# oxli-bio/oxli

Hardware: NVIDIA B200
Metric: canonical k-mers counted/sec (higher is better)
Workload: dtype u64

## Files before the change

oxli_b200/csrc/capi.cu:

```cuda
#include <algorithm>
#include <atomic>
#include <cerrno>
#include <chrono>
#include <cmath>
#include <cstdarg>
#include <cstddef>
#include <condition_variable>
#include <cstdio>
#include <cstdlib>
#include <cstring>
#include <functional>
#include <memory>
#include <mutex>
#include <string>
#include <system_error>
#include <thread>
#include <vector>

#include <fcntl.h>
#include <unistd.h>

#include <cuda_runtime.h>
#include <nvtx3/nvToolsExt.h>

// ... 262 lines not shown
}

int grid_for(const DeviceCtx *c, uint64_t items, int threads, int per_sm) {
    uint64_t want = (items + threads - 1) / threads;
    return (int)std::max<uint64_t>(1, std::min<uint64_t>(want, (uint64_t)c->sms * per_sm));
}

constexpr uint64_t kSparseBytes = 128ull << 20;
uint64_t capacity_for_keys(uint64_t keys);
bool over_loaded(uint64_t size, uint64_t cap) {
    if (cap * 16 < kSparseBytes) return size * 10 > cap * 3;
    return size * 10 > cap * 7;
}

uint64_t pow2_at_least(uint64_t x) {
    uint64_t c = kMinCap;
    while (c < x) c <<= 1;
    return c;
}

uint64_t capacity_for_keys(uint64_t keys) {
    uint64_t cap = pow2_at_least(keys + keys / 2 + 1);
    while (cap * 16 < kSparseBytes && keys * 10 > cap * 3) cap <<= 1;
    return cap;
}

uint64_t slots_for(uint64_t keys) { return std::max(capacity_for_keys(keys), pow2_at_least(keys * 2)); }

oxg_status free_device_bytes(size_t *free_b) {
    size_t total = 0;
    CU(cudaMemGetInfo(free_b, &total));
    return OXG_OK;
}

oxg_status larger_and_fits(uint64_t keys, uint64_t cap, bool *yes) {
    *yes = false;
    const uint64_t want = slots_for(keys);
    if (want <= cap) return OXG_OK;
    size_t free_b = 0;
    TRY(free_device_bytes(&free_b));
    *yes = want * 16 < free_b / 2;
    return OXG_OK;
}


}

namespace {
struct PartPlan {
    uint32_t n_parts = 0, part_bits = 0;
    int n_ranks = 1, self_rank = 0, owner_shift = 64;
    uint32_t grid_a = 0;
    uint32_t frag_cap = 0;
    uint32_t line_shift = 4;
    uint64_t spill_cap = 0;
    uint32_t groups = 1;
    uint32_t n_dest() const { return n_parts * (uint32_t)n_ranks; }
    uint64_t frag_entries() const { return (uint64_t)n_dest() * grid_a * frag_cap; }
};

}

struct oxg_table {
    DeviceCtx *ctx = nullptr;
    uint32_t k = 0;
    ulonglong2 *slots = nullptr;
    uint64_t cap = 0;
    Ctrl *d_ctrl = nullptr;
    Ctrl *h_ctrl = nullptr;
    uint64_t size = 0;
    bool hinted = false;
    uint64_t hint_keys = 0;
    bool pooled = false;
    float last_ms_a = 0.f, last_ms_b = 0.f;
    struct {
        bool active = false;
        PartPlan pl;
        uint32_t launches = 0;
        uint64_t windows = 0, planned = 0;
    } pend;
    uint64_t part_budget = 0;
    uint32_t group_cap = 0;
    uint32_t *d_sketch = nullptr;
    uint32_t *h_sketch = nullptr;
    uint64_t sketch_covers = 0;
    uint64_t est_keys = 0;
    uint64_t last_made = 0;
    uint64_t last_new = 0;
    float last_ms = 0.f;
    uint64_t last_launches = 0;
};

namespace {

TableView view_of(const oxg_table *t, const DeferLists *defer = nullptr) {
    TableView v;
    v.slots = t->slots;
    v.cap = t->cap;
    uint32_t lg = 0;
    while ((1ull << lg) < t->cap) ++lg;
    v.shift = 64 - lg;
    v.limit = t->cap - t->cap / 5;
    v.ctrl = t->d_ctrl;
    v.overflow = defer ? defer->d_pairs : nullptr;
    v.overflow_cap = defer ? defer->cap : 0;
    return v;
}
// ... 144 lines not shown
}

template <int MODE>
oxg_status launch_consume(oxg_table *t, const ConsumeParams &p) {
    DeviceCtx *c = t->ctx;
    const int k = (int)t->k;
    auto grid_of = [&](const void *fn, size_t smem) {
        int per_sm = 1;
        if (cudaOccupancyMaxActiveBlocksPerMultiprocessor(&per_sm, fn, kThreads, smem) != cudaSuccess || per_sm < 1) per_sm = 1;
        const uint64_t tiles_per_cta = specialised_k(t->k) ? kThreads / 32 : 1;
        const uint64_t work = p.n_tiles;
        return (int)std::max<uint64_t>(1, std::min<uint64_t>((work + tiles_per_cta - 1) / tiles_per_cta, (uint64_t)c->sms * per_sm));
    };
    if (const void *fn = specialised_entry(t->k, MODE)) {
        const size_t dyn = consume_dyn_smem(MODE);
        if (dyn) TRY(max_dyn_smem(fn, c->dev, dyn));
        void *args[] = {const_cast<ConsumeParams *>(&p)};
        CU(cudaLaunchKernel(fn, dim3(grid_of(fn, dyn)), dim3(kThreads), args, dyn, c->stream));
    } else {
        const size_t smem = generic_smem_bytes(k);
        consume_generic_kernel<MODE><<<grid_of((const void *)consume_generic_kernel<MODE>, smem), kThreads, smem, c->stream>>>(p);
    }
    LAUNCHED();
    CU(cudaGetLastError());
    return OXG_OK;
}



uint32_t group_launches(const oxg_table *t) {
    const uint32_t g = g_accumulate.load();
    return t->group_cap ? std::min(g, t->group_cap) : g;
}

bool use_partitioned(const oxg_table *t, uint64_t span) {
    if (!specialised_entry(t->k, kModePart)) return false;
    const int choice = g_pipeline.load();
    if (choice == 1) return false;
    if (choice == 2) return true;
    if (t->pend.active) return true;
    return span >= kPartMinWindows;
}

uint32_t choose_parts(const oxg_table *t, uint32_t max_parts) {
    const uint32_t forced = g_parts_override.load();
    if (forced >= 2 && !(forced & (forced - 1))) return std::min(forced, std::max(max_parts, 2u));
    const uint64_t est = std::max(t->size + t->last_new, t->hint_keys);
    if (est == 0) return std::min<uint32_t>(1024, max_parts);
    uint64_t parts = 64;
    while (parts < max_parts && parts * 6144 < est) parts <<= 1;
    return (uint32_t)std::min<uint64_t>(parts, max_parts);
}

size_t scatter_smem_rt(uint32_t k, uint32_t n_dest, uint32_t line_shift) {
    const uint32_t q = 8 * ((k + 7 + 7) / 8);
    const uint32_t bl = ((kWarpTile - 8 + q) + 15) / 16 * 16;
    return (((size_t)n_dest * ((8u << line_shift) + 12) + 16 + 15) & ~(size_t)15) + (size_t)kScatWarps * (2 * bl + 128);
}

oxg_status plan_partitioned(oxg_table *t, uint64_t span, uint64_t n_tiles, int n_ranks, int self_rank, PartPlan *out) {
    DeviceCtx *c = t->ctx;
    PartPlan pl;
    pl.n_parts = choose_parts(t, std::max(2u, 2048u / (uint32_t)n_ranks));
    while ((1u << pl.part_bits) < pl.n_parts) ++pl.part_bits;
    pl.n_ranks = n_ranks; pl.self_rank = self_rank;
    int lg = 0;
    while ((1 << lg) < n_ranks) ++lg;
    pl.owner_shift = 64 - lg;
    pl.line_shift = 4;
    while (pl.line_shift > 1 && scatter_smem_rt(t->k, pl.n_dest(), pl.line_shift) * kScatCtasPerSm > 220u * 1024) --pl.line_shift;
    if (scatter_smem_rt(t->k, pl.n_dest(), pl.line_shift) * kScatCtasPerSm > 220u * 1024) return fail(OXG_ERR_INVALID, "internal: too many scatter destinations");
    const uint64_t tiles_per_cta = kScatWarps;
    pl.grid_a = (uint32_t)std::max<uint64_t>(1, std::min<uint64_t>((n_tiles + tiles_per_cta - 1) / tiles_per_cta, (uint64_t)c->sms * kScatCtasPerSm));
    const uint64_t line = 1ull << pl.line_shift;
    const uint64_t fair = span / ((uint64_t)pl.n_dest() * pl.grid_a) + 1;
    uint64_t sq = 1;
    while (sq * sq < fair) ++sq;
    pl.frag_cap = (uint32_t)((fair + fair / 2 + 4 * sq + line + line - 1) & ~(line - 1));
    pl.spill_cap = span;
    const uint32_t forced_groups = g_groups_override.load();
    pl.groups = forced_groups ? forced_groups : std::max<uint32_t>(1, std::min<uint32_t>(8, (4u * (uint32_t)c->sms + pl.n_parts - 1) / pl.n_parts));
    if (pl.frag_entries() >> 32) return fail(OXG_ERR_INVALID, "internal: fragment buffer too large for one launch");
    *out = pl;
    return OXG_OK;
}

oxg_status scatter_attr(DeviceCtx *c, uint32_t k) { return max_dyn_smem(specialised_entry(k, kModePart), c->dev, 227 * 1024); }

oxg_status ensure_part_buffers(DeviceCtx *c, const PartPlan &pl) {
    TRY(ensure_dev(&c->d_frag, &c->frag_cap, pl.frag_entries()));
    TRY(ensure_dev(&c->d_frag_cnt, &c->frag_cnt_cap, (uint64_t)pl.n_dest() * pl.grid_a));
    TRY(ensure_dev(&c->d_spill, &c->spill_cap, pl.spill_cap));
    if (!c->d_spill_n) CU(cudaMalloc(&c->d_spill_n, 8));
    return OXG_OK;
}

oxg_status launch_part_a(oxg_table *t, ConsumeParams p, const PartPlan &pl, uint64_t *d_frag, uint32_t *d_frag_cnt,
                         uint64_t *d_spill, unsigned long long *d_spill_n, cudaStream_t stream, bool append = false) {
    DeviceCtx *c = t->ctx;
    const void *fn = specialised_entry(t->k, kModePart);
    TRY(scatter_attr(c, t->k));
    const size_t dyn = scatter_smem_rt(t->k, pl.n_dest(), pl.line_shift);
    p.frag = d_frag; p.frag_cnt = d_frag_cnt; p.frag_cap = pl.frag_cap;
    p.n_parts = pl.n_parts; p.part_shift = 64 - pl.part_bits; p.n_dest = pl.n_dest(); p.line_shift = pl.line_shift;
    p.n_ranks = pl.n_ranks; p.self_rank = pl.self_rank; p.owner_shift = pl.owner_shift;
    p.spill = d_spill; p.spill_cap = pl.spill_cap; p.spill_n = d_spill_n;
    p.frag_append = append ? 1u : 0u;
    if (!append) CU(cudaMemsetAsync(d_spill_n, 0, 8, stream));
    void *args[] = {&p};
    CU(cudaLaunchKernel(fn, dim3(pl.grid_a), dim3(kScatThreads), args, dyn, stream));
    LAUNCHED();
    CU(cudaGetLastError());
    return OXG_OK;
}

constexpr int kAggThreadsDirect = 1024;
const void *const kAggCached = (const void *)aggregate_kernel<kAggThreadsDefault, true>;
const void *const kAggDirect = (const void *)aggregate_kernel<kAggThreadsDirect, false>;

uint32_t use_cache_for(const oxg_table *t, const PartPlan &pl, uint64_t windows) {
    const uint64_t keys = std::max(std::max(t->size, t->hint_keys), t->est_keys);
    return keys == 0 || (windows >= 2 * keys && keys <= 8192ull * pl.n_parts) ? 1u : 0u;
}

uint32_t aggregate_groups(const PartPlan &pl, uint32_t use_cache, uint64_t hashes) {
    if (use_cache || g_groups_override.load()) return pl.groups;
    const uint64_t items = std::max<uint64_t>(1, hashes / 40960);
    return (uint32_t)std::max<uint64_t>(pl.groups, std::min<uint64_t>(64, (items + pl.n_parts - 1) / pl.n_parts));
}

AggParams agg_params(const TableView &v, const PartPlan &pl, const AggSource *src, int n_src) {
    AggParams a{};
    a.table = v;
    for (int s = 0; s < n_src; ++s) a.src[s] = src[s];
    a.n_src = n_src;
    a.n_parts = pl.n_parts; a.dest0 = (uint32_t)pl.self_rank * pl.n_parts; a.n_ctas = pl.grid_a;
    a.frag_cap = pl.frag_cap; a.part_bits = pl.part_bits; a.spill_cap = pl.spill_cap;
    a.owner_shift = pl.owner_shift; a.self_rank = pl.self_rank; a.n_ranks = pl.n_ranks;
    return a;
}

oxg_status launch_part_b(oxg_table *t, const TableView &v, const PartPlan &pl, const AggSource *src, int n_src,
                         uint64_t windows, cudaStream_t stream) {
    DeviceCtx *c = t->ctx;
    AggParams a = agg_params(v, pl, src, n_src);
    a.work_counter = (unsigned long long *)&t->d_ctrl->absorb_counter;
    a.use_cache = use_cache_for(t, pl, windows);
    a.groups = aggregate_groups(pl, a.use_cache, windows);
    const void *fn = a.use_cache ? kAggCached : kAggDirect;
    const int threads = a.use_cache ? kAggThreadsDefault : kAggThreadsDirect;
    const size_t smem = aggregate_smem_bytes(a.use_cache != 0);
    if (a.use_cache) TRY(max_dyn_smem(fn, c->dev, smem));
    int per_sm = 1;
    if (cudaOccupancyMaxActiveBlocksPerMultiprocessor(&per_sm, fn, threads, smem) != cudaSuccess || per_sm < 1) per_sm = 1;
    const uint64_t items = (uint64_t)a.n_parts * a.groups;
    const int grid = (int)std::max<uint64_t>(1, std::min<uint64_t>(items, (uint64_t)c->sms * per_sm));
    void *args[] = {&a};
    CU(cudaLaunchKernel(fn, dim3(grid), dim3(threads), args, smem, stream));
    LAUNCHED();
    CU(cudaGetLastError());
// ... 1097 lines not shown
```

oxli_b200/csrc/capi_shard.inc:

```

constexpr int kSnapRing = 8;

struct oxg_shard {
    oxg_table *table = nullptr;
    DeviceCtx *ctx = nullptr;
    int rank = 0, n_ranks = 1;
    PartPlan plan;
    uint64_t round_windows = 0;
    uint64_t small_round = 0;
    uint64_t batch_windows = 0;
    uint8_t *area = nullptr;
    uint64_t area_bytes = 0;
    uint64_t off_gather = 0, off_cnt[2] = {}, off_spill_n[2] = {}, off_frag[2] = {}, off_spill[2] = {};
    uint8_t *peer[kShardMaxRanks] = {};
    bool peer_ipc[kShardMaxRanks] = {};
    bool connected = false;
    uint64_t rounds_done = 0;
    uint64_t gather_seq = 0;
    uint8_t *d_blob = nullptr;
    uint8_t *h_blob = nullptr;
    Ctrl *h_snap[kSnapRing] = {};
    cudaEvent_t ev_round[kSnapRing] = {};
    uint64_t snaps_seen = 0;
    StageRing ring;
// ... 1000 lines not shown
    return OXG_OK;
}

oxg_status shard_dump(oxg_shard *s, const char *path, int sort_mode) {
    if (!s->connected) return fail(OXG_ERR_INVALID, "shard is not connected to its peers (oxg_shard_connect)");
    if (sort_mode < 0 || sort_mode > 2) return fail(OXG_ERR_INVALID, "sort_mode must be 0, 1 or 2");
    if (!path) return fail(OXG_ERR_INVALID, "null argument");
    CallBufs bufs(s->stream);
    LocalPairs lp;
    LocalText tx;
    std::vector<uint64_t> count, len, bytes, start, at;
    oxg_status st = shard_local_pairs(s, bufs, sort_mode, true, &lp);
    local_runs(lp, sort_mode, &count, &len);
    if (st == OXG_OK) st = shard_text_lengths(s, bufs, lp, len, &tx);
    bytes.assign(len.size(), 0);
    if (st == OXG_OK)
        for (size_t j = 0; j < len.size(); ++j) bytes[j] = tx.bounds[j + 1] - tx.bounds[j];
    uint64_t total_n = 0, total_b = 0;
    TRY(shard_place_runs(s, st, sort_mode, path_hash_of(path), count, len, bytes, &start, &at, &total_n, &total_b));
    TRY(shard_agree(s, s->rank == 0 ? create_sized(path, total_b) : OXG_OK));
    const int fd = open(path, O_WRONLY | O_CLOEXEC);
    if (fd < 0) {
        st = fail(OXG_ERR_IO, "cannot open %s: %s", path, strerror(errno));
    } else {
        st = shard_write_text(s, lp, tx, at, fd, path);
        if (close(fd) != 0 && st == OXG_OK) st = fail(OXG_ERR_IO, "cannot write %s: %s", path, strerror(errno));
    }
    cudaStreamSynchronize(s->ring.copy);
    cudaStreamSynchronize(s->stream);
    return shard_agree(s, st);
}

}

extern "C" {

oxg_status oxg_shard_create(int device, uint32_t ksize, int rank, int n_ranks, uint64_t capacity_hint,
                            uint64_t round_windows, oxg_shard **out) {
    if (!out) return fail(OXG_ERR_INVALID, "out is null");
    *out = nullptr;
    if (n_ranks < 1 || n_ranks > kShardMaxRanks || (n_ranks & (n_ranks - 1)))
        return fail(OXG_ERR_INVALID, "n_ranks must be a power of two in 1..%d", kShardMaxRanks);
    if (rank < 0 || rank >= n_ranks) return fail(OXG_ERR_INVALID, "rank out of range");
    if (!specialised_entry(ksize, kModePart)) return fail(OXG_ERR_INVALID, "a sharded table needs a k with a specialised kernel (csrc/klist.h); got %u", ksize);
    auto s = std::make_unique<oxg_shard>();
    TRY(oxg_table_create(device, ksize, capacity_hint, &s->table));
    oxg_table *t = s->table;
    DeviceCtx *c = t->ctx;
    s->ctx = c; s->rank = rank; s->n_ranks = n_ranks;
    std::lock_guard<std::mutex> lk(c->mu);
    CU(cudaSetDevice(c->dev));
    s->round_windows = round_windows ? round_windows : kLaunchWindows;
    if (s->round_windows < (1u << 16)) s->round_windows = 1u << 16;
    s->round_windows = std::max<uint64_t>(s->round_windows, (uint64_t)c->sms * kScatCtasPerSm * kScatWarps * kWarpTile);
    s->round_windows = align_up(s->round_windows, kWarpTile);
    TRY(plan_partitioned(t, s->round_windows, s->round_windows / kWarpTile + 1, n_ranks, rank, &s->plan));
    if (s->plan.grid_a != (uint32_t)(c->sms * kScatCtasPerSm)) return fail(OXG_ERR_INVALID, "internal: round too small for a full grid");
    if (s->plan.spill_cap < lookup_cap(s.get())) return fail(OXG_ERR_INVALID, "internal: spill region smaller than a merge round");
    shard_layout(s.get());
    CU(cudaMalloc(&s->area, s->area_bytes));
    CU(cudaMemsetAsync(s->area, 0, sizeof(ShardHeader) + (uint64_t)n_ranks * kGatherBytes, c->stream));
    CU(cudaStreamCreateWithFlags(&s->stream, cudaStreamNonBlocking));
    TRY(s->ring.init());
    CU(cudaMalloc(&s->d_blob, kGatherBytes));
    CU(cudaMallocHost(&s->h_blob, (uint64_t)n_ranks * kGatherBytes));
    for (int b = 0; b < kSnapRing; ++b) {
        CU(cudaMallocHost(&s->h_snap[b], sizeof(Ctrl)));
        memset(s->h_snap[b], 0, sizeof(Ctrl));
        CU(cudaEventCreateWithFlags(&s->ev_round[b], cudaEventDisableTiming));
    }
    CU(cudaEventCreate(&s->ev_t0));
    CU(cudaEventCreate(&s->ev_t1));
    s->small_round = align_up(std::max<uint64_t>(std::min<uint64_t>(s->round_windows, kLaunchWindows), (uint64_t)s->plan.grid_a * kScatWarps * kWarpTile), kWarpTile);
    s->small_round = std::min(s->small_round, s->round_windows);
    s->batch_windows = s->round_windows;
    s->defer.cap = s->defer.cap2 = std::max<uint64_t>(kShardDeferCap, 2 * s->small_round);
    s->defer.fixed = true;
    CU(cudaMalloc(&s->defer.d_pairs, s->defer.cap * sizeof(ulonglong2)));
    CU(cudaMalloc(&s->defer.d_pairs2, s->defer.cap2 * sizeof(ulonglong2)));
    t->pooled = true;
    {
        cudaMemPool_t pool;
        CU(cudaDeviceGetDefaultMemPool(&pool, c->dev));
        uint64_t keep = ~0ULL;
        CU(cudaMemPoolSetAttribute(pool, cudaMemPoolAttrReleaseThreshold, &keep));
    }
    TRY(s->ring.reserve(kStageBufs, std::min<uint64_t>(s->round_windows, 4ull << 20) + 256 + 16, false, s->stream));
    for (int b = 0; b < kStageBufs; ++b) TRY(s->ring.reserve_offs(b, 1, s->stream));
    CU(cudaMalloc(&t->d_sketch, kSketchRegs * 4));
    CU(cudaMallocHost(&t->h_sketch, kSketchRegs * 4));
    CU(cudaMemsetAsync(t->d_sketch, 0, kSketchRegs * 4, c->stream));
    s->tile_first_cap = s->round_windows / kWarpTile + 4;
    CU(cudaMalloc(&s->d_tile_first, s->tile_first_cap * 8));
    CU(cudaMalloc(&s->d_bins, (uint64_t)n_ranks * c->sms * kRouteCtasPerSm * 4));
    CU(cudaMallocHost(&s->h_list, kLookupStage * 8));
    TRY(scatter_attr(c, ksize));
    for (const void *fn : {(const void *)route_count_kernel<RouteList>, (const void *)route_count_kernel<RouteSlots>,
                           (const void *)route_scan_kernel, (const void *)route_queries_kernel<RouteList>,
                           (const void *)route_queries_kernel<RouteSlots>, (const void *)answer_queries_kernel,
                           (const void *)gather_answers_kernel, (const void *)apply_pairs_kernel,
                           (const void *)erase_walk_segments_kernel, (const void *)erase_mark_segments_kernel,
                           (const void *)erase_rebuild_kernel, (const void *)cut_kernel, (const void *)init_slots_kernel,
                           (const void *)shard_signal_kernel, (const void *)shard_wait_kernel,
                           (const void *)shard_scatter_blob_kernel, (const void *)stats_kernel,
                           (const void *)export_count_kernel, (const void *)export_scan_kernel,
                           (const void *)export_write_kernel, (const void *)radix_hist_kernel,
                           (const void *)radix_scan_kernel, (const void *)radix_scatter_kernel,
                           (const void *)dump_length_kernel, (const void *)dump_bounds_kernel,
                           (const void *)dump_format_kernel}) {
        cudaFuncAttributes attr;
        CU(cudaFuncGetAttributes(&attr, fn));
    }
    TRY(max_dyn_smem(kAggCached, c->dev, aggregate_smem_bytes(true)));
    CU(cudaStreamSynchronize(c->stream));
    s->peer[rank] = s->area;
    s->connected = n_ranks == 1;
    *out = s.release();
    return OXG_OK;
}

oxg_status oxg_shard_destroy(oxg_shard *s) {
    if (!s) return OXG_OK;
    {
        std::lock_guard<std::mutex> lk(s->ctx->mu);
        cudaSetDevice(s->ctx->dev);
        if (s->d_pos) cudaFreeAsync(s->d_pos, s->stream);
// ... 281 lines not shown
```

oxli_b200/csrc/consume.cuh:

```cuda
#pragma once
#include <utility>

#include "hashing.cuh"
#include "table.cuh"

namespace oxg {

template <class F, int... I>
__device__ __forceinline__ void static_for_impl(F &&f, std::integer_sequence<int, I...>) {
    (f(std::integral_constant<int, I>{}), ...);
}
template <int N, class F>
__device__ __forceinline__ void static_for(F &&f) {
    static_for_impl(f, std::make_integer_sequence<int, N>{});
}

#ifndef OXG_MIN_CTAS
#define OXG_MIN_CTAS 3
#endif

constexpr int kTileW = 2048;
constexpr int kThreads = 256;
constexpr int kWPT = kTileW / kThreads;
static_assert(kWPT == 8, "bit-mask extraction assumes 8 windows per thread");
constexpr int kWarpTile = 32 * kWPT;
constexpr int kMaxRanks = 16;

enum Mode : int {
    kModeCount = 0,
    kModeHash = 1,
    kModeFirstBad = 2,
    kModePart = 3
};

struct ConsumeParams {
    const uint8_t *bases;
    uint64_t g0;
    uint64_t w_lo, w_hi;
    uint64_t data_end;
    uint64_t tile_base;
    uint64_t n_tiles;
    const uint64_t *offsets;
    uint64_t n_off;
    const uint64_t *tile_first;
    TableView table;
    uint64_t *hashes_out;
    uint32_t ksize;
    int owner_shift;
    int self_rank;
    int n_ranks;
    uint64_t *frag;
    uint32_t *frag_cnt;
    uint32_t frag_cap;
    uint32_t n_parts;
    uint32_t part_shift;
    uint32_t n_dest;
    uint32_t line_shift;
    uint32_t frag_append;
    uint64_t *spill;
    uint64_t spill_cap;
    unsigned long long *spill_n;
};

static __global__ void tile_first_kernel(const uint64_t *__restrict__ offsets, uint64_t n_off,
                                  uint64_t tile_base, uint64_t n_tiles, uint32_t tile_w,
                                  uint64_t *__restrict__ tile_first) {
    uint64_t t = blockIdx.x * (uint64_t)blockDim.x + threadIdx.x;
    if (t >= n_tiles) return;
    const uint64_t want = tile_base + t * tile_w + 1;
    uint64_t lo = 0, hi = n_off;
    while (lo < hi) {
        uint64_t mid = (lo + hi) >> 1;
        if (offsets[mid] < want) lo = mid + 1; else hi = mid;
    }
    tile_first[t] = lo;
}

__device__ __forceinline__ uint4 load_bases16(const ConsumeParams &p, uint64_t g) {
    if (g + 16 <= p.data_end) {
        return __ldcs(reinterpret_cast<const uint4 *>(p.bases + (g - p.g0)));
    }
    uint32_t w[4] = {0x4e4e4e4eu, 0x4e4e4e4eu, 0x4e4e4e4eu, 0x4e4e4e4eu};
    for (int b = 0; b < 16; ++b) {
        if (g + b < p.data_end) {
            uint32_t c = p.bases[g + b - p.g0];
            w[b >> 2] = (w[b >> 2] & ~(0xffu << (8 * (b & 3)))) | (c << (8 * (b & 3)));
        }
    }
    return make_uint4(w[0], w[1], w[2], w[3]);
}

template <int BL>
__device__ __forceinline__ void stage16_raw(const ConsumeParams &p, uint64_t w0, int v, uint4 raw, uint8_t *s_fw,
                                            uint8_t *s_rc, uint16_t *s_bad) {
    const uint64_t g = w0 + 16ull * v;
    uint32_t u[4] = {upper4(raw.x), upper4(raw.y), upper4(raw.z), upper4(raw.w)};
    uint32_t ok = acgt_mask4(u[0]) | (acgt_mask4(u[1]) << 4) | (acgt_mask4(u[2]) << 8) |
                  (acgt_mask4(u[3]) << 12);
    if (g + 16 > p.data_end) {
        uint32_t keep = g >= p.data_end ? 0u : (0xffffu >> (16 - (uint32_t)(p.data_end - g)));
        ok &= keep;
    }
    *reinterpret_cast<uint4 *>(s_fw + 16 * v) = make_uint4(u[0], u[1], u[2], u[3]);
    *reinterpret_cast<uint4 *>(s_rc + BL - 16 - 16 * v) =
        make_uint4(bswap32(complement4(u[3])), bswap32(complement4(u[2])),
                   bswap32(complement4(u[1])), bswap32(complement4(u[0])));
    s_bad[v] = (uint16_t)(~ok);
}

template <int BL>
// ... 557 lines not shown
```

oxli_b200/csrc/scatter.cuh:

```cuda
#pragma once
#include "consume.cuh"

namespace oxg {

#ifndef OXG_SCAT_THREADS
#define OXG_SCAT_THREADS 384
#endif
#ifndef OXG_SCAT_CTAS
#define OXG_SCAT_CTAS 2
#endif
constexpr int kScatThreads = OXG_SCAT_THREADS;
constexpr int kScatCtasPerSm = OXG_SCAT_CTAS;
constexpr int kScatWarps = kScatThreads / 32;

template <int K>
struct ScatWarpBuf {
    static constexpr int BL = TileGeom<K>::BL;
    static constexpr int kBytes = 2 * BL + 64 + 64;
};

template <int K>
inline size_t scatter_smem_bytes(uint32_t n_dest, uint32_t line_shift) {
    return (((size_t)n_dest * ((8u << line_shift) + 12) + 16 + 15) & ~(size_t)15) + (size_t)kScatWarps * ScatWarpBuf<K>::kBytes;
}

template <int K>
__global__ void __launch_bounds__(kScatThreads, kScatCtasPerSm) scatter_kernel(const ConsumeParams p) {
    using G = TileGeom<K>;
    constexpr int BL = G::BL, NV = G::NV, NE = G::NE;
    static_assert(NV + 8 <= 32 && NE <= 16, "per-warp mask buffers are 64 bytes each");
    extern __shared__ __align__(128) uint8_t sm[];
    const uint32_t nd = p.n_dest, ls = p.line_shift, line = 1u << ls;
    uint64_t *stage = reinterpret_cast<uint64_t *>(sm);
    uint2 *book = reinterpret_cast<uint2 *>(sm + ((size_t)nd << (ls + 3)));
    uint32_t *flist = reinterpret_cast<uint32_t *>(book + nd);
    uint32_t *s_nflush = flist + nd;
    uint8_t *wbuf = sm + ((((size_t)nd * ((8u << ls) + 12) + 16) + 15) & ~(size_t)15) + (size_t)(threadIdx.x >> 5) * ScatWarpBuf<K>::kBytes;
    uint8_t *s_fw = wbuf, *s_rc = wbuf + BL;
    uint16_t *s_bad = reinterpret_cast<uint16_t *>(wbuf + 2 * BL);
    uint32_t *s_end = reinterpret_cast<uint32_t *>(wbuf + 2 * BL + 64);

    const int lane = threadIdx.x & 31, warp = threadIdx.x >> 5;
    const uint64_t frag_row = (uint64_t)gridDim.x * p.frag_cap;
    uint64_t *const my_frag = p.frag + (uint64_t)blockIdx.x * p.frag_cap;
    for (uint32_t i = threadIdx.x; i < nd; i += kScatThreads) {
        const uint32_t at = p.frag_append ? p.frag_cnt[(uint64_t)i * gridDim.x + blockIdx.x] : 0u;
        book[i] = make_uint2(at, at);
    }
    if (threadIdx.x == 0) *s_nflush = 0;
    __syncthreads();

    auto dest_of = [&](uint64_t h) {
        uint32_t d = (uint32_t)((h * kPhi) >> p.part_shift);
        if (p.n_ranks > 1) d += (uint32_t)(h >> p.owner_shift) * p.n_parts;
        return d;
    };

    uint64_t n_counted = 0, first_bad_unused = ~0ULL;
    const uint64_t tiles_per_round = (uint64_t)gridDim.x * kScatWarps;
    const uint64_t n_rounds = (p.n_tiles + tiles_per_round - 1) / tiles_per_round;
    auto tile_of = [&](uint64_t r) { return (r * gridDim.x + blockIdx.x) * kScatWarps + warp; };

    uint4 raw = make_uint4(0, 0, 0, 0);
    uint64_t tf = 0, off = ~0ULL;
    auto fetch = [&](uint64_t t, uint4 &raw_, uint64_t &tf_) {
        if (t < p.n_tiles) {
            if (lane < NV) raw_ = load_bases16(p, p.tile_base + t * kWarpTile + 16ull * lane);
            tf_ = __ldg(p.tile_first + t);
        }
    };
    auto fetch_off = [&](uint64_t t, uint64_t tf_) {
        const uint64_t rr = tf_ + lane;
        return (t < p.n_tiles && rr < p.n_off) ? __ldg(p.offsets + rr) : ~0ULL;
    };
    fetch(tile_of(0), raw, tf);
    off = fetch_off(tile_of(0), tf);

    const uint32_t lanes_per_line = ls >= 2 ? (line >> 2) : 1u;

    for (uint64_t r = 0; r < n_rounds; ++r) {
        const uint64_t t = tile_of(r);
        uint4 raw_next = make_uint4(0, 0, 0, 0);
        uint64_t tf_next = 0;
        fetch(tile_of(r + 1), raw_next, tf_next);
        uint64_t h[kWPT] = {};
        if (t < p.n_tiles) {
            const uint64_t w0 = p.tile_base + t * kWarpTile;
            if (lane < NE) s_end[lane] = 0;
            __syncwarp();
            if (lane < NV) stage16_raw<BL>(p, w0, lane, raw, s_fw, s_rc, s_bad);
            {
                const uint64_t e = off - 1 - w0;
                if (e < (uint64_t)BL) atomicOr(&s_end[e >> 5], 1u << (e & 31));
                if (__shfl_sync(0xffffffffu, e < (uint64_t)BL, 31)) {
                    for (uint64_t q = tf + 32 + lane; q < p.n_off; q += 32) {
                        const uint64_t e2 = p.offsets[q] - 1 - w0;
                        if (e2 >= (uint64_t)BL) break;
                        atomicOr(&s_end[e2 >> 5], 1u << (e2 & 31));
                    }
                }
            }
            __syncwarp();
            const uint32_t valid = lane_valid_mask<K, kModePart>(p, s_bad, s_end, w0, lane, first_bad_unused);
            if (valid) lane_hashes<K>(s_fw, s_rc, lane * kWPT, valid, h);
        }
        const uint64_t off_next = fetch_off(tile_of(r + 1), tf_next);

        uint32_t dst[kWPT], q[kWPT];
#pragma unroll
        for (int j = 0; j < kWPT; ++j) {
            dst[j] = 0; q[j] = 0;
            if (h[j] != 0) { ++n_counted; dst[j] = dest_of(h[j]); q[j] = atomicAdd(&book[dst[j]].y, 1u); }
        }
        __syncthreads();

        uint32_t later = 0, spilled = 0, last = 0;
        uint2 bk[kWPT];
#pragma unroll
        for (int j = 0; j < kWPT; ++j) bk[j] = book[dst[j]];
#pragma unroll
        for (int j = 0; j < kWPT; ++j) {
            if (h[j] == 0) continue;
            const uint2 b = bk[j];
            const uint32_t total = min(b.y, p.frag_cap), line_end = (b.x & ~(line - 1)) + line;
            if (q[j] >= total) { spilled |= 1u << j; continue; }
            if (q[j] + 1 == total) last |= 1u << j;
            if (q[j] < line_end) {
                stage[((size_t)dst[j] << ls) + (q[j] & (line - 1))] = h[j];
                if (q[j] + 1 == line_end) flist[atomicAdd(s_nflush, 1u)] = dst[j];
            } else if (q[j] < (total & ~(line - 1))) my_frag[dst[j] * frag_row + q[j]] = h[j];
            else later |= 1u << j;
        }
        if (__any_sync(0xffffffffu, spilled != 0)) {
            const uint32_t mine = __popc(spilled);
            uint32_t incl = mine;
            for (int o = 1; o < 32; o <<= 1) {
                const uint32_t v = __shfl_up_sync(0xffffffffu, incl, o);
                if (lane >= o) incl += v;
            }
            const uint32_t tot = __shfl_sync(0xffffffffu, incl, 31);
            unsigned long long base = 0;
            if (lane == 0) base = atomicAdd(p.spill_n, (unsigned long long)tot);
            base = __shfl_sync(0xffffffffu, base, 0) + (incl - mine);
#pragma unroll
            for (int j = 0; j < kWPT; ++j)
                if ((spilled >> j) & 1u) { if (base < p.spill_cap) p.spill[base] = h[j]; ++base; }
        }
        __syncthreads();

        {
            const uint32_t n_flush = *s_nflush;
            if (ls >= 2) {
                const uint32_t per_warp = 32u / lanes_per_line, sub = lane / lanes_per_line, li = (lane % lanes_per_line) * 4;
                for (uint32_t e = warp * per_warp + sub; e < n_flush; e += kScatWarps * per_warp) {
                    const uint32_t d = flist[e];
                    const uint64_t *src = stage + ((size_t)d << ls) + li;
                    const ulonglong2 v0 = *reinterpret_cast<const ulonglong2 *>(src), v1 = *reinterpret_cast<const ulonglong2 *>(src + 2);
                    uint64_t *dstp = my_frag + d * frag_row + (book[d].x & ~(line - 1)) + li;
                    asm volatile("st.global.v4.u64 [%0], {%1,%2,%3,%4};" ::"l"(dstp), "l"(v0.x), "l"(v0.y), "l"(v1.x), "l"(v1.y) : "memory");
                }
            } else {
                const uint32_t per_warp = 32u >> ls, sub = lane >> ls, li = lane & (line - 1);
                for (uint32_t e = warp * per_warp + sub; e < n_flush; e += kScatWarps * per_warp) {
                    const uint32_t d = flist[e];
                    my_frag[d * frag_row + (book[d].x & ~(line - 1)) + li] = stage[((size_t)d << ls) + li];
                }
            }
        }
        __syncthreads();

#pragma unroll
        for (int j = 0; j < kWPT; ++j) {
            if ((later >> j) & 1u) stage[((size_t)dst[j] << ls) + (q[j] & (line - 1))] = h[j];
            if ((last >> j) & 1u) book[dst[j]].x = q[j] + 1;
        }
        if (threadIdx.x == 0) *s_nflush = 0;
        raw = raw_next; tf = tf_next; off = off_next;
    }

    __syncthreads();
    {
        const uint32_t per_warp = 32u >> ls, sub = lane >> ls, li = lane & (line - 1);
        for (uint32_t d = warp * per_warp + sub; d < nd; d += kScatWarps * per_warp) {
            const uint32_t pos = book[d].x, part = pos & (line - 1);
            if (part) my_frag[d * frag_row + (pos - part) + li] = li < part ? stage[((size_t)d << ls) + li] : 0ull;
        }
        for (uint32_t d = threadIdx.x; d < nd; d += kScatThreads)
            p.frag_cnt[(uint64_t)d * gridDim.x + blockIdx.x] = min((book[d].x + line - 1) & ~(line - 1), p.frag_cap);
    }
    for (int o = 16; o; o >>= 1) n_counted += __shfl_xor_sync(0xffffffffu, n_counted, o);
    if (lane == 0 && n_counted) atomicAdd((unsigned long long *)&p.table.ctrl->counted, (unsigned long long)n_counted);
}

}
```

Before: 41.30 billion.

## Replace per-destination line staging with batched counting-sort scatter in pass A

The scatter kernel no longer stages hashes in per-destination shared-memory lines with flush lists. It buffers up to three tiles per warp, counts per destination, prefix-sums the counts across the CTA, and reorders hashes into a shared batch sorted by destination. It then writes them to fragments with contiguous, coalesced stores. This removes the per-round book/line bookkeeping and partial-line padding, at the cost of extra block-wide syncs and a scan per batch, and it caps destinations at 2048 and tiles at 2^31.

```diff
diff --git a/oxli_b200/csrc/capi.cu b/oxli_b200/csrc/capi.cu
--- a/oxli_b200/csrc/capi.cu
+++ b/oxli_b200/csrc/capi.cu
@@ -338,7 +338,7 @@
     int n_ranks = 1, self_rank = 0, owner_shift = 64;
     uint32_t grid_a = 0;
     uint32_t frag_cap = 0;
-    uint32_t line_shift = 4;
+    uint32_t batch_tiles = 1;
     uint64_t spill_cap = 0;
     uint32_t groups = 1;
     uint32_t n_dest() const { return n_parts * (uint32_t)n_ranks; }
@@ -589,10 +589,15 @@
     return (uint32_t)std::min<uint64_t>(parts, max_parts);
 }
 
-size_t scatter_smem_rt(uint32_t k, uint32_t n_dest, uint32_t line_shift) {
+size_t scatter_smem_rt(uint32_t k, uint32_t n_dest, uint32_t batch_tiles) {
     const uint32_t q = 8 * ((k + 7 + 7) / 8);
     const uint32_t bl = ((kWarpTile - 8 + q) + 15) / 16 * 16;
-    return (((size_t)n_dest * ((8u << line_shift) + 12) + 16 + 15) & ~(size_t)15) + (size_t)kScatWarps * (2 * bl + 128);
+    return scatter_smem_bytes(n_dest, batch_tiles, (int)(2 * bl + 128));
+}
+
+uint64_t scatter_full_grid_tiles(const DeviceCtx *c) { return (uint64_t)c->sms * kScatCtasPerSm * kScatWarps; }
+uint32_t scatter_grid(const DeviceCtx *c, uint64_t n_tiles) {
+    return (uint32_t)std::max<uint64_t>(1, std::min<uint64_t>((n_tiles + kScatWarps - 1) / kScatWarps, (uint64_t)c->sms * kScatCtasPerSm));
 }
 
 oxg_status plan_partitioned(oxg_table *t, uint64_t span, uint64_t n_tiles, int n_ranks, int self_rank, PartPlan *out) {
@@ -604,16 +609,15 @@
     int lg = 0;
     while ((1 << lg) < n_ranks) ++lg;
     pl.owner_shift = 64 - lg;
-    pl.line_shift = 4;
-    while (pl.line_shift > 1 && scatter_smem_rt(t->k, pl.n_dest(), pl.line_shift) * kScatCtasPerSm > 220u * 1024) --pl.line_shift;
-    if (scatter_smem_rt(t->k, pl.n_dest(), pl.line_shift) * kScatCtasPerSm > 220u * 1024) return fail(OXG_ERR_INVALID, "internal: too many scatter destinations");
-    const uint64_t tiles_per_cta = kScatWarps;
-    pl.grid_a = (uint32_t)std::max<uint64_t>(1, std::min<uint64_t>((n_tiles + tiles_per_cta - 1) / tiles_per_cta, (uint64_t)c->sms * kScatCtasPerSm));
-    const uint64_t line = 1ull << pl.line_shift;
+    pl.batch_tiles = kScatMaxBatchTiles;
+    while (pl.batch_tiles > 1 && scatter_smem_rt(t->k, pl.n_dest(), pl.batch_tiles) * kScatCtasPerSm > 220u * 1024) --pl.batch_tiles;
+    if (scatter_smem_rt(t->k, pl.n_dest(), pl.batch_tiles) * kScatCtasPerSm > 220u * 1024) return fail(OXG_ERR_INVALID, "internal: too many scatter destinations");
+    pl.grid_a = scatter_grid(c, n_tiles);
+    if (pl.grid_a * (uint64_t)kMaxSources > kAggMaxFrags) return fail(OXG_ERR_INVALID, "internal: more pass A CTAs than pass B can take");
     const uint64_t fair = span / ((uint64_t)pl.n_dest() * pl.grid_a) + 1;
     uint64_t sq = 1;
     while (sq * sq < fair) ++sq;
-    pl.frag_cap = (uint32_t)((fair + fair / 2 + 4 * sq + line + line - 1) & ~(line - 1));
+    pl.frag_cap = (uint32_t)((fair + fair / 2 + 4 * sq + 3) & ~(uint64_t)3);
     pl.spill_cap = span;
     const uint32_t forced_groups = g_groups_override.load();
     pl.groups = forced_groups ? forced_groups : std::max<uint32_t>(1, std::min<uint32_t>(8, (4u * (uint32_t)c->sms + pl.n_parts - 1) / pl.n_parts));
@@ -637,12 +641,13 @@
     DeviceCtx *c = t->ctx;
     const void *fn = specialised_entry(t->k, kModePart);
     TRY(scatter_attr(c, t->k));
-    const size_t dyn = scatter_smem_rt(t->k, pl.n_dest(), pl.line_shift);
+    const size_t dyn = scatter_smem_rt(t->k, pl.n_dest(), pl.batch_tiles);
     p.frag = d_frag; p.frag_cnt = d_frag_cnt; p.frag_cap = pl.frag_cap;
-    p.n_parts = pl.n_parts; p.part_shift = 64 - pl.part_bits; p.n_dest = pl.n_dest(); p.line_shift = pl.line_shift;
+    p.n_parts = pl.n_parts; p.part_shift = 64 - pl.part_bits; p.n_dest = pl.n_dest(); p.batch_tiles = pl.batch_tiles;
     p.n_ranks = pl.n_ranks; p.self_rank = pl.self_rank; p.owner_shift = pl.owner_shift;
     p.spill = d_spill; p.spill_cap = pl.spill_cap; p.spill_n = d_spill_n;
     p.frag_append = append ? 1u : 0u;
+    if (p.n_tiles >> 31) return fail(OXG_ERR_INVALID, "internal: too many tiles for one pass A launch");
     if (!append) CU(cudaMemsetAsync(d_spill_n, 0, 8, stream));
     void *args[] = {&p};
     CU(cudaLaunchKernel(fn, dim3(pl.grid_a), dim3(kScatThreads), args, dyn, stream));
diff --git a/oxli_b200/csrc/capi_shard.inc b/oxli_b200/csrc/capi_shard.inc
--- a/oxli_b200/csrc/capi_shard.inc
+++ b/oxli_b200/csrc/capi_shard.inc
@@ -1076,10 +1076,10 @@
     CU(cudaSetDevice(c->dev));
     s->round_windows = round_windows ? round_windows : kLaunchWindows;
     if (s->round_windows < (1u << 16)) s->round_windows = 1u << 16;
-    s->round_windows = std::max<uint64_t>(s->round_windows, (uint64_t)c->sms * kScatCtasPerSm * kScatWarps * kWarpTile);
+    s->round_windows = std::max<uint64_t>(s->round_windows, scatter_full_grid_tiles(c) * kWarpTile);
     s->round_windows = align_up(s->round_windows, kWarpTile);
     TRY(plan_partitioned(t, s->round_windows, s->round_windows / kWarpTile + 1, n_ranks, rank, &s->plan));
-    if (s->plan.grid_a != (uint32_t)(c->sms * kScatCtasPerSm)) return fail(OXG_ERR_INVALID, "internal: round too small for a full grid");
+    if (s->plan.grid_a != scatter_grid(c, scatter_full_grid_tiles(c))) return fail(OXG_ERR_INVALID, "internal: round too small for a full grid");
     if (s->plan.spill_cap < lookup_cap(s.get())) return fail(OXG_ERR_INVALID, "internal: spill region smaller than a merge round");
     shard_layout(s.get());
     CU(cudaMalloc(&s->area, s->area_bytes));
@@ -1095,7 +1095,7 @@
     }
     CU(cudaEventCreate(&s->ev_t0));
     CU(cudaEventCreate(&s->ev_t1));
-    s->small_round = align_up(std::max<uint64_t>(std::min<uint64_t>(s->round_windows, kLaunchWindows), (uint64_t)s->plan.grid_a * kScatWarps * kWarpTile), kWarpTile);
+    s->small_round = align_up(std::max<uint64_t>(std::min<uint64_t>(s->round_windows, kLaunchWindows), scatter_full_grid_tiles(c) * kWarpTile), kWarpTile);
     s->small_round = std::min(s->small_round, s->round_windows);
     s->batch_windows = s->round_windows;
     s->defer.cap = s->defer.cap2 = std::max<uint64_t>(kShardDeferCap, 2 * s->small_round);
diff --git a/oxli_b200/csrc/consume.cuh b/oxli_b200/csrc/consume.cuh
--- a/oxli_b200/csrc/consume.cuh
+++ b/oxli_b200/csrc/consume.cuh
@@ -55,7 +55,7 @@
     uint32_t n_parts;
     uint32_t part_shift;
     uint32_t n_dest;
-    uint32_t line_shift;
+    uint32_t batch_tiles;
     uint32_t frag_append;
     uint64_t *spill;
     uint64_t spill_cap;
diff --git a/oxli_b200/csrc/scatter.cuh b/oxli_b200/csrc/scatter.cuh
--- a/oxli_b200/csrc/scatter.cuh
+++ b/oxli_b200/csrc/scatter.cuh
@@ -12,6 +12,8 @@
 constexpr int kScatThreads = OXG_SCAT_THREADS;
 constexpr int kScatCtasPerSm = OXG_SCAT_CTAS;
 constexpr int kScatWarps = kScatThreads / 32;
+constexpr int kScatMaxBatchTiles = 3;
+static_assert(kScatWarps * 256 >= 2048, "step 2 scans 256 destinations per warp, up to 2048 of them");
 
 template <int K>
 struct ScatWarpBuf {
@@ -19,35 +21,38 @@
     static constexpr int kBytes = 2 * BL + 64 + 64;
 };
 
-template <int K>
-inline size_t scatter_smem_bytes(uint32_t n_dest, uint32_t line_shift) {
-    return (((size_t)n_dest * ((8u << line_shift) + 12) + 16 + 15) & ~(size_t)15) + (size_t)kScatWarps * ScatWarpBuf<K>::kBytes;
+__host__ __device__ inline size_t scatter_dest_bytes(uint32_t n_dest) { return ((size_t)n_dest * 12 + 15) & ~(size_t)15; }
+__host__ __device__ inline size_t scatter_smem_bytes(uint32_t n_dest, uint32_t batch_tiles, int warp_buf_bytes) {
+    return (size_t)kScatWarps * batch_tiles * kWarpTile * 8 + scatter_dest_bytes(n_dest) + 16 + (size_t)kScatWarps * warp_buf_bytes;
 }
 
 template <int K>
 __global__ void __launch_bounds__(kScatThreads, kScatCtasPerSm) scatter_kernel(const ConsumeParams p) {
     using G = TileGeom<K>;
     constexpr int BL = G::BL, NV = G::NV, NE = G::NE;
+    constexpr int kMaxPerLane = kScatMaxBatchTiles * kWPT;
     static_assert(NV + 8 <= 32 && NE <= 16, "per-warp mask buffers are 64 bytes each");
     extern __shared__ __align__(128) uint8_t sm[];
-    const uint32_t nd = p.n_dest, ls = p.line_shift, line = 1u << ls;
-    uint64_t *stage = reinterpret_cast<uint64_t *>(sm);
-    uint2 *book = reinterpret_cast<uint2 *>(sm + ((size_t)nd << (ls + 3)));
-    uint32_t *flist = reinterpret_cast<uint32_t *>(book + nd);
-    uint32_t *s_nflush = flist + nd;
-    uint8_t *wbuf = sm + ((((size_t)nd * ((8u << ls) + 12) + 16) + 15) & ~(size_t)15) + (size_t)(threadIdx.x >> 5) * ScatWarpBuf<K>::kBytes;
+    const int lane = threadIdx.x & 31, warp = threadIdx.x >> 5;
+    const uint32_t nd = p.n_dest, slice = p.batch_tiles * kWarpTile;
+    uint64_t *batch = reinterpret_cast<uint64_t *>(sm);
+    uint32_t *cnt = reinterpret_cast<uint32_t *>(batch + (size_t)kScatWarps * slice);
+    uint32_t *pos = cnt + nd, *to_frag = pos + nd;
+    uint32_t *s_total = reinterpret_cast<uint32_t *>(reinterpret_cast<uint8_t *>(cnt) + scatter_dest_bytes(nd));
+    unsigned long long *s_counted = reinterpret_cast<unsigned long long *>(s_total + 2);
+    uint8_t *wbuf = reinterpret_cast<uint8_t *>(s_total + 4) + (size_t)warp * ScatWarpBuf<K>::kBytes;
     uint8_t *s_fw = wbuf, *s_rc = wbuf + BL;
     uint16_t *s_bad = reinterpret_cast<uint16_t *>(wbuf + 2 * BL);
     uint32_t *s_end = reinterpret_cast<uint32_t *>(wbuf + 2 * BL + 64);
-
-    const int lane = threadIdx.x & 31, warp = threadIdx.x >> 5;
-    const uint64_t frag_row = (uint64_t)gridDim.x * p.frag_cap;
+    uint64_t *const my_slice = batch + (size_t)warp * slice;
+
+    const uint32_t frag_row = gridDim.x * p.frag_cap;
     uint64_t *const my_frag = p.frag + (uint64_t)blockIdx.x * p.frag_cap;
     for (uint32_t i = threadIdx.x; i < nd; i += kScatThreads) {
-        const uint32_t at = p.frag_append ? p.frag_cnt[(uint64_t)i * gridDim.x + blockIdx.x] : 0u;
-        book[i] = make_uint2(at, at);
+        to_frag[i] = p.frag_append ? p.frag_cnt[(uint64_t)i * gridDim.x + blockIdx.x] : 0u;
+        cnt[i] = 0; pos[i] = 0;
     }
-    if (threadIdx.x == 0) *s_nflush = 0;
+    if (threadIdx.x == 0) *s_counted = 0;
     __syncthreads();
 
     auto dest_of = [&](uint64_t h) {
@@ -56,140 +61,146 @@
         return d;
     };
 
-    uint64_t n_counted = 0, first_bad_unused = ~0ULL;
-    const uint64_t tiles_per_round = (uint64_t)gridDim.x * kScatWarps;
-    const uint64_t n_rounds = (p.n_tiles + tiles_per_round - 1) / tiles_per_round;
-    auto tile_of = [&](uint64_t r) { return (r * gridDim.x + blockIdx.x) * kScatWarps + warp; };
+    uint64_t first_bad_unused = ~0ULL;
+    const uint32_t n_tiles = (uint32_t)p.n_tiles, tiles_per_round = gridDim.x * kScatWarps;
+    const uint32_t n_rounds = (n_tiles + tiles_per_round - 1) / tiles_per_round;
+    const uint32_t R = p.batch_tiles, n_batches = (n_rounds + R - 1) / R;
+    auto tile_of = [&](uint32_t r) { return (r * gridDim.x + blockIdx.x) * kScatWarps + warp; };
 
     uint4 raw = make_uint4(0, 0, 0, 0);
     uint64_t tf = 0, off = ~0ULL;
-    auto fetch = [&](uint64_t t, uint4 &raw_, uint64_t &tf_) {
-        if (t < p.n_tiles) {
-            if (lane < NV) raw_ = load_bases16(p, p.tile_base + t * kWarpTile + 16ull * lane);
+    auto fetch = [&](uint32_t t, uint4 &raw_, uint64_t &tf_) {
+        if (t < n_tiles) {
+            if (lane < NV) raw_ = load_bases16(p, p.tile_base + (uint64_t)t * kWarpTile + 16ull * lane);
             tf_ = __ldg(p.tile_first + t);
         }
     };
-    auto fetch_off = [&](uint64_t t, uint64_t tf_) {
+    auto fetch_off = [&](uint32_t t, uint64_t tf_) {
         const uint64_t rr = tf_ + lane;
-        return (t < p.n_tiles && rr < p.n_off) ? __ldg(p.offsets + rr) : ~0ULL;
+        return (t < n_tiles && rr < p.n_off) ? __ldg(p.offsets + rr) : ~0ULL;
     };
     fetch(tile_of(0), raw, tf);
     off = fetch_off(tile_of(0), tf);
 
-    const uint32_t lanes_per_line = ls >= 2 ? (line >> 2) : 1u;
-
-    for (uint64_t r = 0; r < n_rounds; ++r) {
-        const uint64_t t = tile_of(r);
-        uint4 raw_next = make_uint4(0, 0, 0, 0);
-        uint64_t tf_next = 0;
-        fetch(tile_of(r + 1), raw_next, tf_next);
-        uint64_t h[kWPT] = {};
-        if (t < p.n_tiles) {
-            const uint64_t w0 = p.tile_base + t * kWarpTile;
-            if (lane < NE) s_end[lane] = 0;
+    for (uint32_t b = 0; b < n_batches; ++b) {
+        const uint32_t r0 = b * R, n_here = min(r0 + R, n_rounds) - r0;
+
+        for (uint32_t i = 0; i < n_here; ++i) {
+            const uint32_t r = r0 + i, t = tile_of(r);
+            uint4 raw_next = make_uint4(0, 0, 0, 0);
+            uint64_t tf_next = 0;
+            fetch(tile_of(r + 1), raw_next, tf_next);
+            uint64_t h[kWPT] = {};
+            if (t < n_tiles) {
+                const uint64_t w0 = p.tile_base + (uint64_t)t * kWarpTile;
+                if (lane < NE) s_end[lane] = 0;
+                __syncwarp();
+                if (lane < NV) stage16_raw<BL>(p, w0, lane, raw, s_fw, s_rc, s_bad);
+                {
+                    const uint64_t e = off - 1 - w0;
+                    if (e < (uint64_t)BL) atomicOr(&s_end[e >> 5], 1u << (e & 31));
+                    if (__shfl_sync(0xffffffffu, e < (uint64_t)BL, 31)) {
+                        for (uint64_t q = tf + 32 + lane; q < p.n_off; q += 32) {
+                            const uint64_t e2 = p.offsets[q] - 1 - w0;
+                            if (e2 >= (uint64_t)BL) break;
+                            atomicOr(&s_end[e2 >> 5], 1u << (e2 & 31));
+                        }
+                    }
+                }
+                __syncwarp();
+                const uint32_t valid = lane_valid_mask<K, kModePart>(p, s_bad, s_end, w0, lane, first_bad_unused);
+                if (valid) lane_hashes<K>(s_fw, s_rc, lane * kWPT, valid, h);
+            }
+            off = fetch_off(tile_of(r + 1), tf_next);
+            raw = raw_next; tf = tf_next;
+#pragma unroll
+            for (int j = 0; j < kWPT; ++j) {
+                if (h[j] != 0) atomicAdd(&cnt[dest_of(h[j])], 1u);
+                my_slice[i * kWarpTile + j * 32 + lane] = h[j];
+            }
             __syncwarp();
-            if (lane < NV) stage16_raw<BL>(p, w0, lane, raw, s_fw, s_rc, s_bad);
-            {
-                const uint64_t e = off - 1 - w0;
-                if (e < (uint64_t)BL) atomicOr(&s_end[e >> 5], 1u << (e & 31));
-                if (__shfl_sync(0xffffffffu, e < (uint64_t)BL, 31)) {
-                    for (uint64_t q = tf + 32 + lane; q < p.n_off; q += 32) {
-                        const uint64_t e2 = p.offsets[q] - 1 - w0;
-                        if (e2 >= (uint64_t)BL) break;
-                        atomicOr(&s_end[e2 >> 5], 1u << (e2 & 31));
-                    }
-                }
-            }
-            __syncwarp();
-            const uint32_t valid = lane_valid_mask<K, kModePart>(p, s_bad, s_end, w0, lane, first_bad_unused);
-            if (valid) lane_hashes<K>(s_fw, s_rc, lane * kWPT, valid, h);
-        }
-        const uint64_t off_next = fetch_off(tile_of(r + 1), tf_next);
-
-        uint32_t dst[kWPT], q[kWPT];
-#pragma unroll
-        for (int j = 0; j < kWPT; ++j) {
-            dst[j] = 0; q[j] = 0;
-            if (h[j] != 0) { ++n_counted; dst[j] = dest_of(h[j]); q[j] = atomicAdd(&book[dst[j]].y, 1u); }
-        }
-        __syncthreads();
-
-        uint32_t later = 0, spilled = 0, last = 0;
-        uint2 bk[kWPT];
-#pragma unroll
-        for (int j = 0; j < kWPT; ++j) bk[j] = book[dst[j]];
-#pragma unroll
-        for (int j = 0; j < kWPT; ++j) {
-            if (h[j] == 0) continue;
-            const uint2 b = bk[j];
-            const uint32_t total = min(b.y, p.frag_cap), line_end = (b.x & ~(line - 1)) + line;
-            if (q[j] >= total) { spilled |= 1u << j; continue; }
-            if (q[j] + 1 == total) last |= 1u << j;
-            if (q[j] < line_end) {
-                stage[((size_t)dst[j] << ls) + (q[j] & (line - 1))] = h[j];
-                if (q[j] + 1 == line_end) flist[atomicAdd(s_nflush, 1u)] = dst[j];
-            } else if (q[j] < (total & ~(line - 1))) my_frag[dst[j] * frag_row + q[j]] = h[j];
-            else later |= 1u << j;
-        }
-        if (__any_sync(0xffffffffu, spilled != 0)) {
-            const uint32_t mine = __popc(spilled);
-            uint32_t incl = mine;
+        }
+        __syncthreads();
+
+        if (warp * 256u < nd) {
+            const uint32_t lo = warp * 256u;
+            uint32_t carry = 0;
+            for (uint32_t d = lane; d < lo; d += 32) carry += cnt[d];
+            carry = __reduce_add_sync(0xffffffffu, carry);
+            uint32_t v[8], x[8];
+#pragma unroll
+            for (int u = 0; u < 8; ++u) {
+                const uint32_t d = lo + 32 * u + lane;
+                v[u] = d < nd ? cnt[d] : 0u;
+                x[u] = v[u];
+            }
+#pragma unroll
             for (int o = 1; o < 32; o <<= 1) {
-                const uint32_t v = __shfl_up_sync(0xffffffffu, incl, o);
-                if (lane >= o) incl += v;
-            }
-            const uint32_t tot = __shfl_sync(0xffffffffu, incl, 31);
-            unsigned long long base = 0;
-            if (lane == 0) base = atomicAdd(p.spill_n, (unsigned long long)tot);
-            base = __shfl_sync(0xffffffffu, base, 0) + (incl - mine);
-#pragma unroll
-            for (int j = 0; j < kWPT; ++j)
-                if ((spilled >> j) & 1u) { if (base < p.spill_cap) p.spill[base] = h[j]; ++base; }
-        }
-        __syncthreads();
-
-        {
-            const uint32_t n_flush = *s_nflush;
-            if (ls >= 2) {
-                const uint32_t per_warp = 32u / lanes_per_line, sub = lane / lanes_per_line, li = (lane % lanes_per_line) * 4;
-                for (uint32_t e = warp * per_warp + sub; e < n_flush; e += kScatWarps * per_warp) {
-                    const uint32_t d = flist[e];
-                    const uint64_t *src = stage + ((size_t)d << ls) + li;
-                    const ulonglong2 v0 = *reinterpret_cast<const ulonglong2 *>(src), v1 = *reinterpret_cast<const ulonglong2 *>(src + 2);
-                    uint64_t *dstp = my_frag + d * frag_row + (book[d].x & ~(line - 1)) + li;
-                    asm volatile("st.global.v4.u64 [%0], {%1,%2,%3,%4};" ::"l"(dstp), "l"(v0.x), "l"(v0.y), "l"(v1.x), "l"(v1.y) : "memory");
-                }
-            } else {
-                const uint32_t per_warp = 32u >> ls, sub = lane >> ls, li = lane & (line - 1);
-                for (uint32_t e = warp * per_warp + sub; e < n_flush; e += kScatWarps * per_warp) {
-                    const uint32_t d = flist[e];
-                    my_frag[d * frag_row + (book[d].x & ~(line - 1)) + li] = stage[((size_t)d << ls) + li];
-                }
-            }
-        }
-        __syncthreads();
-
-#pragma unroll
-        for (int j = 0; j < kWPT; ++j) {
-            if ((later >> j) & 1u) stage[((size_t)dst[j] << ls) + (q[j] & (line - 1))] = h[j];
-            if ((last >> j) & 1u) book[dst[j]].x = q[j] + 1;
-        }
-        if (threadIdx.x == 0) *s_nflush = 0;
-        raw = raw_next; tf = tf_next; off = off_next;
+#pragma unroll
+                for (int u = 0; u < 8; ++u) {
+                    const uint32_t y = __shfl_up_sync(0xffffffffu, x[u], o);
+                    if (lane >= o) x[u] += y;
+                }
+            }
+#pragma unroll
+            for (int u = 0; u < 8; ++u) {
+                const uint32_t d = lo + 32 * u + lane;
+                if (d < nd) {
+                    const uint32_t start = carry + x[u] - v[u], fill = min(to_frag[d] + pos[d], p.frag_cap);
+                    pos[d] = start; to_frag[d] = fill - start;
+                }
+                carry += __shfl_sync(0xffffffffu, x[u], 31);
+            }
+            if (lane == 0 && lo + 256u >= nd) { *s_total = carry; *s_counted += carry; }
+        }
+        uint64_t v[kMaxPerLane];
+#pragma unroll
+        for (int u = 0; u < kMaxPerLane; ++u) v[u] = u < (int)(n_here * kWPT) ? my_slice[u * 32 + lane] : 0ull;
+        __syncthreads();
+
+        for (uint32_t d = threadIdx.x; d < nd; d += kScatThreads) cnt[d] = 0;
+#pragma unroll
+        for (int u = 0; u < kMaxPerLane; ++u)
+            if (v[u] != 0) batch[atomicAdd(&pos[dest_of(v[u])], 1u)] = v[u];
+        __syncthreads();
+
+        const uint32_t total = *s_total;
+        for (uint32_t i0 = warp * 128; i0 < total; i0 += kScatThreads * 4) {
+            uint64_t h[4];
+#pragma unroll
+            for (int u = 0; u < 4; ++u) {
+                const uint32_t i = i0 + 32 * u + lane;
+                h[u] = i < total ? batch[i] : 0ull;
+            }
+            uint32_t spilled = 0;
+#pragma unroll
+            for (int u = 0; u < 4; ++u) {
+                if (h[u] == 0) continue;
+                const uint32_t d = dest_of(h[u]), at = i0 + 32 * u + lane + to_frag[d];
+                if (at < p.frag_cap) my_frag[d * frag_row + at] = h[u];
+                else spilled |= 1u << u;
+            }
+            if (__any_sync(0xffffffffu, spilled != 0)) {
+                const uint32_t mine = __popc(spilled);
+                uint32_t incl = mine;
+                for (int o = 1; o < 32; o <<= 1) {
+                    const uint32_t y = __shfl_up_sync(0xffffffffu, incl, o);
+                    if (lane >= o) incl += y;
+                }
+                unsigned long long base = 0;
+                if (lane == 31) base = atomicAdd(p.spill_n, (unsigned long long)incl);
+                base = __shfl_sync(0xffffffffu, base, 31) + (incl - mine);
+#pragma unroll
+                for (int u = 0; u < 4; ++u)
+                    if ((spilled >> u) & 1u) { if (base < p.spill_cap) p.spill[base] = h[u]; ++base; }
+            }
+        }
+        __syncthreads();
     }
 
-    __syncthreads();
-    {
-        const uint32_t per_warp = 32u >> ls, sub = lane >> ls, li = lane & (line - 1);
-        for (uint32_t d = warp * per_warp + sub; d < nd; d += kScatWarps * per_warp) {
-            const uint32_t pos = book[d].x, part = pos & (line - 1);
-            if (part) my_frag[d * frag_row + (pos - part) + li] = li < part ? stage[((size_t)d << ls) + li] : 0ull;
-        }
-        for (uint32_t d = threadIdx.x; d < nd; d += kScatThreads)
-            p.frag_cnt[(uint64_t)d * gridDim.x + blockIdx.x] = min((book[d].x + line - 1) & ~(line - 1), p.frag_cap);
-    }
-    for (int o = 16; o; o >>= 1) n_counted += __shfl_xor_sync(0xffffffffu, n_counted, o);
-    if (lane == 0 && n_counted) atomicAdd((unsigned long long *)&p.table.ctrl->counted, (unsigned long long)n_counted);
+    for (uint32_t d = threadIdx.x; d < nd; d += kScatThreads)
+        p.frag_cnt[(uint64_t)d * gridDim.x + blockIdx.x] = min(to_frag[d] + pos[d], p.frag_cap);
+    if (threadIdx.x == 0 && *s_counted) atomicAdd((unsigned long long *)&p.table.ctrl->counted, *s_counted);
 }
 
 }
```

Result: faster. 42.92 billion, median of 6 (+3.9%).
